# JoshuaLim007/Software-Raytracer

Hardware: AMD Instinct MI355X
Metric: path-samples/sec at 1920x1080x8-bounce; achieved HBM GB/s vs peak (higher is better)
Workload: dtype f32; 1 GPU; BASELINE config 2: Scene1.json 1920x1080, 32 spp, 8 bounces, FOV 55, camera at origin; workload_key=Scene1 1920x1080 rows0-1080 spp32 b8, partition=single frame

## Files before the change

### software-raytracer_amd/csrc/srt_capi.hip

```cpp
#include <hip/hip_runtime.h>
#include <math.h>
#include <stdarg.h>
#include <stddef.h>
#include <stdio.h>
#include <stdlib.h>
#include <string.h>

#include <algorithm>
#include <exception>
#include <new>
#include <vector>

#include "srt_kernel.hip.h"
#include "srt_gbuffer.hip.h"
#include "srt_denoise.hip.h"
#include "srt_temporal.hip.h"
#include "srt_upsample.hip.h"
#include "srt_antialias.hip.h"
#include "srt_variance.hip.h"
#include "srt_moments.hip.h"
#include "srt_refit.hip.h"
#include "srt_rays.hip.h"
#include "srt_outputs_host.h"
#include "srt_rays_host.h"
// ... 1111 lines not shown
template <int MIN_WAVES, bool MESH>
static void launch_pathtrace(bool tally, bool in_lds, bool multi, bool defer, dim3 grid, size_t lds_bytes, hipStream_t stream, const srt::KernelParams& K) {
    using srt::pathtrace_kernel;
    void (*const kernel)(srt::KernelParams) =
        tally && defer    ? pathtrace_kernel<MIN_WAVES, MESH, true, false, true, false, true>
        : tally && multi  ? pathtrace_kernel<MIN_WAVES, MESH, true, true, false, false, true>
        : tally           ? pathtrace_kernel<MIN_WAVES, MESH, true, false, false, false, true>
        : in_lds && defer ? pathtrace_kernel<MIN_WAVES, MESH, true, false, true>
        : in_lds && multi ? pathtrace_kernel<MIN_WAVES, MESH, true, true, false>
        : in_lds          ? pathtrace_kernel<MIN_WAVES, MESH, true, false, false>
        : defer           ? pathtrace_kernel<MIN_WAVES, MESH, false, false, true>
        : multi           ? pathtrace_kernel<MIN_WAVES, MESH, false, true, false>
                          : pathtrace_kernel<MIN_WAVES, MESH, false, false, false>;
    hipLaunchKernelGGL(kernel, grid, dim3(srt::WG_THREADS), lds_bytes, stream, K);
}

static void launch_pathtrace_rows(bool tally, bool six, dim3 grid, size_t lds_bytes, hipStream_t stream, const srt::KernelParams& K) {
    using srt::pathtrace_kernel;
    void (*const kernel)(srt::KernelParams) =
        tally ? pathtrace_kernel<5, false, true, false, false, false, true, true>
        : six ? pathtrace_kernel<6, false, true, false, false, false, false, true>
              : pathtrace_kernel<5, false, true, false, false, false, false, true>;
    hipLaunchKernelGGL(kernel, grid, dim3(srt::WG_THREADS), lds_bytes, stream, K);
}

static int launch_render(srt_context* ctx, const srt_render_params* p, srt::KernelParams& K, const KernelSetup& ks, const RenderLaunch& L) {
    const bool in_lds = ctx->scene_in_lds[ks.img];
    const bool want_work = (p->flags & SRT_RENDER_COUNT_WORK) != 0;
    const bool rule_applies = (p->sample_count >= 64 || K.n_tris > 0) && p->sample_count >= 32 && K.steps <= 1;
    const bool tally = ((L.record && rule_applies) || want_work) && in_lds;
    ctx->count_work = want_work;
    ctx->count_work_valid = want_work && tally;
    if (tally && want_work) {
        SRT_HIP(ctx, hipMemsetAsync(ctx->d_work, 0, srt::TALLY_ALL * sizeof(unsigned long long), ctx->stream));
        K.work_counter = ctx->d_work;
    }
    const bool timing = !(p->flags & SRT_RENDER_NO_TIMING);
    if (timing) SRT_HIP(ctx, hipEventRecord(ctx->ev_begin, ctx->stream));
    const bool multi = L.shape.tile_h < srt::TILE_H || (K.steps > 1 && !(K.flags & SRT_RENDER_PREVIEW)) || L.bgrid;
    if (K.n_tris > 0)
        launch_pathtrace<4, true>(tally, in_lds, multi, L.defer, L.grid, ks.lds_bytes, ctx->stream, K);
#ifdef SRT_DEV
    else if (ks.use == 1 && in_lds && !multi && !L.defer && !tally)
        hipLaunchKernelGGL((srt::pathtrace_kernel<4, false>), L.grid, dim3(srt::WG_THREADS), ks.lds_bytes, ctx->stream, K);
    else if (ks.use == 3 && in_lds && !multi && !L.defer && !tally)
        hipLaunchKernelGGL((srt::pathtrace_kernel<3, false>), L.grid, dim3(srt::WG_THREADS), ks.lds_bytes, ctx->stream, K);
#endif
    else if (L.rows) {
        const size_t rows_lds = ks.lds_bytes - (size_t)(srt::WG_SCRATCH_BYTES - srt::WG_SCRATCH_BYTES_ROWS);
        bool six = srt::rows_six_waves(rows_lds);
#ifdef SRT_DEV
        if (ks.use == 5) six = false;
#endif
        launch_pathtrace_rows(tally, six, L.grid, rows_lds, ctx->stream, K);
    }
    else
        launch_pathtrace<5, false>(tally, in_lds, multi, L.defer, L.grid, ks.lds_bytes, ctx->stream, K);
    if (L.defer) {
        SRT_HIP(ctx, hipGetLastError());
        hipLaunchKernelGGL(srt::fold_kernel, dim3((unsigned)L.shape.wg8), dim3(256), 0, ctx->stream, K, (int)L.shape.wg_x);
    }
    SRT_HIP(ctx, hipGetLastError());
    if (timing) SRT_HIP(ctx, hipEventRecord(ctx->ev_end, ctx->stream));
    ctx->pending_timed = timing;
    if (L.record) {
        const size_t nwg = (size_t)L.grid.x * L.grid.y;
        SRT_HIP(ctx, hipMemcpyAsync(ctx->h_wg_cost, ctx->d_wg_cost, REC_WORDS * nwg * 4, hipMemcpyDeviceToHost, ctx->stream));
        SRT_HIP(ctx, hipEventRecord(ctx->ev_cost, ctx->stream));
        ctx->recording = true;
        ctx->rec_gx = L.grid.x, ctx->rec_gy = L.grid.y;
        ctx->rec_has_work = tally;
        ctx->rec_step_w = probe_step_weight(K, ProbeWeights());
        ctx->order_stale = false;
    }
    return SRT_OK;
}

static void note_pending(srt_context* ctx, const srt_render_params* p, const srt::KernelParams& K, const RenderLaunch& L) {
    ctx->launched = true;
    ctx->stats_pending = true;
    ctx->pending_samples = (uint64_t)ctx->width * (uint64_t)K.rows * p->sample_count;
    ctx->pending_chunks = (uint32_t)L.shape.chunks;
    ctx->pending_tile_rows = (uint32_t)L.shape.tile_h;
    ctx->pending_chunk_samples = L.defer ? (uint32_t)L.shape.chunk : 0u;
    ctx->pending_shape_source = L.shape.source;
    ctx->work_layout[0] = K.nu, ctx->work_layout[1] = K.nc, ctx->work_layout[2] = K.K, ctx->work_layout[3] = K.nb;
}

extern "C" {

int srt_render(srt_context* ctx, const srt_render_params* p) {
    if (const int rc = check_render_params(ctx, p)) return rc;
    SRT_HIP(ctx, hipSetDevice(ctx->device));
    srt::KernelParams K;
    const KernelSetup ks = fill_kernel_params(ctx, p, K);
    ctx->count_rays = (p->flags & SRT_RENDER_COUNT_RAYS) != 0;
    if (ctx->count_rays) SRT_HIP(ctx, hipMemsetAsync(ctx->d_rays, 0, sizeof(unsigned long long), ctx->stream));
    RenderLaunch L;
    if (const int rc = enter_band(ctx, K)) return rc;
    if (const int rc = plan_launch(ctx, p, K, ks, L)) return rc;
    if (const int rc = plan_cost_order(ctx, p, K, ks, L)) return rc;
    if (const int rc = launch_render(ctx, p, K, ks, L)) return rc;
    note_pending(ctx, p, K, L);
    return SRT_OK;
}

#ifdef SRT_DEV
// ... 1182 lines not shown
```

### software-raytracer_amd/csrc/srt_kernel.hip.h

```cpp
#pragma once

#include <hip/hip_runtime.h>
#include <stdint.h>

#include <type_traits>

#include "srt_defs.h"
#include "srt_launch_shape.h"

namespace srt {

struct KernelParams {
    float cam_pos[3];
    float right_rd[3];
    float up_ld[3];
    float fwd_clip[3];
    int32_t width, height;
    int32_t y0, rows;
    uint32_t first_sample, sample_count;
    int32_t max_bounces;
    uint32_t seed, flags;
    int32_t steps, stripe_width, selected;
    int32_t bgrid_w, bgrid_h;
    int32_t nu4, nc, K, nsT, nb;
    int32_t nu;
    int32_t off_bounds, off_box, off_mat;
    int32_t scene_vec4;
    const float4* scene;
    const float4* bvh_nodes;
    const float4* bvh_tris;
    const int32_t* bvh_gidpos;
    int32_t n_tris;
    float mesh_center[3];
    float mesh_half[3];
    float mesh_r1;
    float mesh_bs_radius;
    int32_t mesh_defer;
    int32_t mesh_wait;
    int32_t tile_h;
    int32_t chunk;
    int32_t chunk_full;
    float4* sample_rows;
    unsigned long long* tile_masks;
    uint32_t* tile_chain;
    int32_t chunk_layers;
    const uint32_t* wg_order;
    uint32_t* wg_cost;
    uint32_t wg_blocks;
    unsigned long long* work_counter;
    float4* accumulator;
    uint32_t* framebuffer;
    unsigned long long* ray_counter;
#ifdef SRT_DEV
    int32_t chain_mode;
    uint32_t chain_arg;
#endif
};

#ifdef SRT_DEV
enum : int32_t {
    DEV_CHAIN_NATURAL = 0,
    DEV_CHAIN_OFF = 1,
    DEV_CHAIN_CUT = 2,
    DEV_CHAIN_TILES = 3,
};
__host__ __device__ inline uint32_t dev_chain_cut(int32_t mode, uint32_t arg, uint32_t layers, uint32_t tile) {
    if (mode == DEV_CHAIN_CUT) return arg < layers ? arg : layers;
    if (mode == DEV_CHAIN_TILES) return srt_mix32(srt_mix32(arg ^ 0x9E3779B9u) + tile) % (layers + 1u);
    if (mode == DEV_CHAIN_OFF) return 0u;
    return layers;
}
#endif

constexpr uint32_t KF_BLOCK_GRID = 0x10u;
constexpr uint32_t KF_BOXES_FINITE = 0x20u;
constexpr uint32_t SRT_MESH_ORDER_W = 6u;
constexpr int TILE_W = 8, TILE_H = 8;
constexpr int WG_TILES_X = 2, WG_TILES_Y = 2;
constexpr int WG_THREADS = 64 * WG_TILES_X * WG_TILES_Y;
constexpr int WG_W = TILE_W * WG_TILES_X, WG_H = TILE_H * WG_TILES_Y;
struct TilePixel {
    int lx, ly, x, y;
};
__device__ __forceinline__ TilePixel tile_pixel() {
    const int lane = threadIdx.x & 63, wave = threadIdx.x >> 6;
    TilePixel t;
    t.lx = (wave % WG_TILES_X) * TILE_W + (lane & 7), t.ly = (wave / WG_TILES_X) * TILE_H + (lane >> 3);
    t.x = (int)blockIdx.x * WG_W + t.lx, t.y = (int)blockIdx.y * WG_H + t.ly;
    return t;
}
constexpr int WORK_MAX = 512;
constexpr int RING_DEPTH = 2;
constexpr int WAVE_RING_BYTES = 64 * RING_DEPTH * 16;
constexpr int WAVE_SCRATCH_BYTES = 64 * 8 + WORK_MAX * 2 + 64 * 12 * 4 + WAVE_RING_BYTES;
constexpr int WG_SCRATCH_BYTES = WAVE_SCRATCH_BYTES * WG_TILES_X * WG_TILES_Y;
constexpr int ROWS_IN_FLIGHT = 8;
constexpr int WG_SCRATCH_BYTES_ROWS = (WAVE_SCRATCH_BYTES - WAVE_RING_BYTES) * WG_TILES_X * WG_TILES_Y;
constexpr int MESH_Q = 512;
constexpr float MESH_T_MIN_CULL = 0.0099f;
#ifdef SRT_STATS
__device__ unsigned long long g_stats[8];
#define SRT_STAT(i, v) do { if (__builtin_amdgcn_mbcnt_hi(~0u, __builtin_amdgcn_mbcnt_lo(~0u, 0u)) == 0) atomicAdd(&g_stats[i], (unsigned long long)(v)); } while (0)
#else
#define SRT_STAT(i, v) do { } while (0)
#endif
// ... 835 lines not shown

__device__ __forceinline__ void accumulate_sample(const KernelParams& P, float4& acc, RGB c, float a, uint32_t sidx) {
    const uint32_t frame = P.first_sample + sidx;
    if (sidx == 0 && (P.flags & 1u) != 0) {
        acc = make_float4(c.r, c.g, c.b, a);
    } else {
        float weight = frame <= 16777216u ? div_window(1.0f, (float)(int)frame) : (float)(1.0 / (double)(int)frame);
        float om = 1 - weight;
        acc.x = clamp0(acc.x * om) + c.r * weight;
        acc.y = clamp0(acc.y * om) + c.g * weight;
        acc.z = clamp0(acc.z * om) + c.b * weight;
        acc.w = clamp0(acc.w * om) + a * weight;
    }
}
__device__ __forceinline__ uint32_t tone_map(const float4 acc) {
    float r = acc.x / (1.0f + acc.x);
    float g = acc.y / (1.0f + acc.y);
    float b = acc.z / (1.0f + acc.z);
    float a = acc.w / (0.0f + acc.w);
    return pack_channel(a) << 24 | pack_channel(r) << 16 | pack_channel(g) << 8 | pack_channel(b);
}
__device__ __forceinline__ void store_framebuffer(uint32_t* framebuffer, int x, int y, int W, int H, const float4 r) {
    if (framebuffer) framebuffer[(size_t)(H - 1 - y) * W + x] = tone_map(r);
}
__device__ __forceinline__ void store_result(float4* dst, size_t p, uint32_t* framebuffer, int x, int y, int W, int H, const float4 r) {
    dst[p] = r;
    store_framebuffer(framebuffer, x, y, W, H, r);
}
__device__ __forceinline__ void store_pixel(const KernelParams& P, uint32_t pix, const float4 acc) {
    P.accumulator[pix] = acc;
    const uint32_t px = tone_map(acc);
    const uint32_t py = pix / (uint32_t)P.width, pxx = pix - py * (uint32_t)P.width;
    P.framebuffer[(size_t)(P.height - 1 - (int)py) * P.width + pxx] = px;
}

template <bool SCENE_LDS, bool ROWS = false>
__device__ __forceinline__ Lds make_lds(const KernelParams& P, float4* lds, int waves, int wave) {
    constexpr int stride = WAVE_SCRATCH_BYTES - (ROWS ? WAVE_RING_BYTES : 0);
    char* wg = reinterpret_cast<char*>(lds + (SCENE_LDS ? P.scene_vec4 : 0));
    char* scratch = wg + wave * stride;
    const float4* image;
    if constexpr (SCENE_LDS)
        image = lds;
    else
        image = P.scene;
    return Lds{image, image + CONST_ROWS, P.nu4, P.nu, P.nc, P.K, P.nsT, P.nb, P.off_bounds, P.off_box, P.off_mat,
               reinterpret_cast<unsigned long long*>(scratch), reinterpret_cast<unsigned short*>(scratch + 64 * 8),
               reinterpret_cast<float*>(scratch + 64 * 8 + WORK_MAX * 2),
               reinterpret_cast<float4*>(scratch + 64 * 8 + WORK_MAX * 2 + 64 * 12 * 4),
               reinterpret_cast<unsigned*>(wg + waves * stride + wave * MESH_WAVE_BYTES)};
}

template <int MIN_WAVES, bool MESH, bool SCENE_LDS = true, bool MULTI = false, bool DEFER = false, bool PROBE = false, bool TALLY_ = false, bool ROWS = false>
__global__ void __launch_bounds__(WG_THREADS, MIN_WAVES) pathtrace_kernel(const KernelParams P) {
    static_assert(!PROBE || (!MULTI && !DEFER), "the probe runs the full-tile pool");
    static_assert(!ROWS || (!MULTI && !DEFER && !PROBE), "rows of the sample buffer: one chunk, full tiles, a real launch");
    constexpr bool TALLY = TALLY_ || PROBE;
    extern __shared__ float4 lds_scene[];
    Tally<TALLY> tally{};
#if defined(SRT_STATS) && SRT_STATS == 3
    Prof prof;
    prof.last = (long long)__builtin_readcyclecounter();
    for (int i = 0; i < 8; ++i) prof.acc[i] = 0;
#endif
    if constexpr (SCENE_LDS) {
        constexpr int STAGE = 8;
        const int n = P.scene_vec4;
        float4 row[STAGE];
#pragma unroll
        for (int k = 0; k < STAGE; ++k) {
            const int i = (int)threadIdx.x + k * WG_THREADS;
            row[k] = i < n ? P.scene[i] : make_float4(0, 0, 0, 0);
        }
#pragma unroll
        for (int k = 0; k < STAGE; ++k) {
            const int i = (int)threadIdx.x + k * WG_THREADS;
            if (i < n) lds_scene[i] = row[k];
        }
        for (int i = (int)threadIdx.x + STAGE * WG_THREADS; i < n; i += WG_THREADS) lds_scene[i] = P.scene[i];
        __syncthreads();
    }
    const Lds S = make_lds<SCENE_LDS, ROWS>(P, lds_scene, WG_TILES_X * WG_TILES_Y, threadIdx.x >> 6);
    if (PROBE && (threadIdx.x >> 6) != 0) return;

    const int lane = threadIdx.x & 63, wave = threadIdx.x >> 6;
    const int tile_h = P.tile_h;
#if defined(SRT_STATS) && SRT_STATS == 6
    const long long t_start = (long long)__builtin_readcyclecounter();
    const unsigned long long r_start = __builtin_amdgcn_s_memrealtime();
    const unsigned hw_start = __builtin_amdgcn_s_getreg(0xF804), xcc_start = __builtin_amdgcn_s_getreg(0xF814);
#elif defined(SRT_STATS) && SRT_STATS == 5
    const long long t_start = (long long)__builtin_readcyclecounter();
#else
    const long long t_start = !PROBE && P.wg_cost ? (long long)__builtin_amdgcn_s_memrealtime() : 0;
#endif
    uint32_t block_id = blockIdx.y * gridDim.x + blockIdx.x;
    if (P.wg_order) block_id = P.wg_order[block_id];
    const int bx = (int)(block_id % gridDim.x), by = (int)(block_id / gridDim.x);
    const int tx = bx * WG_W + (lane & (TILE_W - 1)) * WG_TILES_X + (wave % WG_TILES_X);
    const int ty = by * (tile_h * WG_TILES_Y) + (lane / TILE_W) * WG_TILES_Y + (wave / WG_TILES_X);
    const int W = P.width, H = P.height;
    const bool bgrid = MULTI && (P.flags & KF_BLOCK_GRID) != 0;
    bool in_range_;
    int x_, y_, ax, ay;
    if (bgrid) {
        const int sw = P.stripe_width > 0 ? P.stripe_width : W;
        const int per_stripe = (sw + P.steps - 1) / P.steps;
        const int stripe = tx / per_stripe;
        ax = stripe * sw + (tx - stripe * per_stripe) * P.steps;
        ay = (P.y0 / P.steps + ty) * P.steps;
        in_range_ = tx < P.bgrid_w && ty < P.bgrid_h && ax < W && ay < P.y0 + P.rows && (lane / TILE_W) < tile_h;
        if (!in_range_) ax = 0, ay = (P.y0 / P.steps) * P.steps;
        x_ = ax, y_ = ay;
    } else {
        in_range_ = tx < W && ty < P.rows && (lane / TILE_W) < tile_h;
        x_ = in_range_ ? tx : 0, y_ = in_range_ ? (P.y0 + ty) : P.y0;
        ax = x_, ay = y_;
        if (P.steps > 1) {
            const int s0 = P.stripe_width > 0 ? (x_ / P.stripe_width) * P.stripe_width : 0;
            ax = s0 + ((x_ - s0) / P.steps) * P.steps;
            ay = (y_ / P.steps) * P.steps;
        }
    }
    const bool in_range = in_range_;
    const int x = x_, y = y_;
    const uint32_t pixel = (uint32_t)(x + y * W);
    const uint32_t rng_pixel = (uint32_t)(ax + ay * W);
    auto write_blocks = [&](bool have, int bx0, int by0, float4 val, bool keep) {
        const unsigned long long m = __builtin_amdgcn_ballot_w64(have);
        if (m == 0ull) return;
        const int n = __builtin_popcountll(m);
        const int rank = (int)__builtin_amdgcn_mbcnt_hi((unsigned)(m >> 32), __builtin_amdgcn_mbcnt_lo((unsigned)m, 0u));
        float4* sv = S.ring;
        unsigned* sa = reinterpret_cast<unsigned*>(S.work);
        __builtin_amdgcn_wave_barrier();
        if (have) {
            sv[rank] = val;
            sa[rank] = (unsigned)bx0, sa[64 + rank] = (unsigned)by0;
            sa[128 + rank] = keep ? 0u : tone_map(val);
        }
        __builtin_amdgcn_wave_barrier();
        const int steps = P.steps, per = steps * steps;
        const int L = per < 64 ? per : 64, G = 64 / L;
        const int g = lane / L, ql = lane - g * L;
        for (int b0 = 0; b0 < n; b0 += G) {
            const int b = b0 + g;
            const bool on = g < G && b < n;
            const int bi = on ? b : 0;
            const int x0 = (int)sa[bi], y0b = (int)sa[64 + bi];
            const float4 v = sv[bi];
            const uint32_t px = sa[128 + bi];
// ... 5 lines not shown
            x_end = x_end < W ? x_end : W;
            int y_hi = y0b + steps;
            y_hi = y_hi < P.y0 + P.rows ? y_hi : P.y0 + P.rows;
            for (int q = ql; q < per; q += 64) {
                const int j = q / steps, i = q - j * steps;
                const int xx = x0 + i, yy = y0b + j;
                if (on && xx < x_end && yy >= P.y0 && yy < y_hi) {
                    const uint32_t pp = (uint32_t)(xx + yy * W);
                    if (keep) {
                        float4 a = P.accumulator[pp];
                        accumulate_sample(P, a, RGB{v.x, v.y, v.z}, tag_alpha(__float_as_uint(v.w)), 0);
                        P.accumulator[pp] = a;
                        P.framebuffer[(size_t)(H - 1 - yy) * W + xx] = tone_map(a);
                    } else {
                        P.accumulator[pp] = v;
                        P.framebuffer[(size_t)(H - 1 - yy) * W + xx] = px;
                    }
                }
            }
        }
        __builtin_amdgcn_wave_barrier();
    };
    int lead_lane = lane;
    if constexpr (MULTI) {
        if (P.steps > 1 && !(P.flags & 4u) && !bgrid) {
            const uint32_t key = in_range ? rng_pixel : 0xFFFFFFFFu - (uint32_t)lane;
            unsigned long long same = 0ull;
            for (int i = 0; i < 64; ++i)
                if ((uint32_t)__builtin_amdgcn_readlane((int)key, i) == key) same |= 1ull << i;
            lead_lane = __builtin_ctzll(same);
        }
    }
    const bool is_leader = lead_lane == lane;

    float nX = ((float)ax / (float)W) * 2 - 1;
    float nY = ((float)ay / (float)H) * 2 - 1;
    V3 u = v3(P.right_rd[0] * nX, P.right_rd[1] * nX, P.right_rd[2] * nX);
    V3 vv = v3(P.up_ld[0] * nY, P.up_ld[1] * nY, P.up_ld[2] * nY);
    const V3 dir0 = normalized(v3((u.x + vv.x) + P.fwd_clip[0], (u.y + vv.y) + P.fwd_clip[1], (u.z + vv.z) + P.fwd_clip[2]));
    const V3 cam = v3(P.cam_pos[0], P.cam_pos[1], P.cam_pos[2]);

    bool parked = false;
    const Hit h0 = closest_hit<MESH, TALLY, SCENE_LDS>(S, P, cam, dir0, true, 1, parked, tally SRT_PROF_ARG);

    const bool reset = (P.flags & 1u) != 0;
    uint32_t s_base = 0u, count = P.sample_count;
    if constexpr (DEFER) {
        const uint32_t z = blockIdx.z, zf = (uint32_t)P.chunk_full, S = (uint32_t)P.chunk, half = S >> 1;
        s_base = SRT_CHUNK_FIRST(z, S, zf, half);
        const uint32_t want = z < zf ? S : half;
        count = P.sample_count - s_base < want ? P.sample_count - s_base : want;
    }
    const int B = P.max_bounces;
    unsigned rays = 0;

    auto accumulate = [&](float4& acc, RGB c, float a, uint32_t sidx) { accumulate_sample(P, acc, c, a, sidx); };
    auto write_pixel = [&](uint32_t pix, const float4 acc) { store_pixel(P, pix, acc); };

    const bool preview = (P.flags & 4u) != 0;
    const bool pix_traced = in_range && h0.prim >= 0 && B > 0 && !preview;
    const bool traced = pix_traced && is_leader;
    float4 untraced_val = make_float4(0, 0, 0, 0);
    tally.add(TALLY_UNTRACED_WAVES, __builtin_amdgcn_ballot_w64(in_range && !pix_traced) != 0ull ? 1u : 0u);
    tally.add(TALLY_WAVES, 1u);
    if (!PROBE && in_range && !pix_traced && (!DEFER || blockIdx.z == 0)) {
        RGB c;
        float ca = 0.0f;
        if (h0.prim < 0) {
            c = environment(S, dir0);
            ca = environment_alpha(dir0);
        } else if (preview) {
            float4 m0 = S.mat(h0.prim, 0), m1 = S.mat(h0.prim, 1);
            float k2 = 2 * dot3(dir0, h0.n);
            const V3 rd = v3(dir0.x - h0.n.x * k2, dir0.y - h0.n.y * k2, dir0.z - h0.n.z * k2);
            RGB refl = environment(S, rd);
            const float k = m0.y, sm = m0.x;
            float fresnal = 0;
            if (S.order(h0.prim) == P.selected) {
                fresnal = 1 - dot3(v3(h0.n.x * -1, h0.n.y * -1, h0.n.z * -1), dir0);
                fresnal = tmax(fresnal, 0.0f);
                if (fresnal < 0.0f) {
                    fresnal = 0;
                } else if (fresnal >= 0.5f) {
                    fresnal = 1;
                } else {
                    fresnal = (fresnal - 0.0f) / (0.5f - 0.0f);
                    fresnal = fresnal * fresnal * (3 - 2 * fresnal);
                }
            }
            RGB base{clamp0(m0.z), clamp0(m0.w), clamp0(m1.x)}, emis{clamp0(m1.y), clamp0(m1.z), clamp0(m1.w)};
            const float omk = 1 - k;
            RGB a{clamp0(clamp0(clamp0(base.r * omk) + clamp0(clamp0(refl.r * k) * sm)) + emis.r),
                  clamp0(clamp0(clamp0(base.g * omk) + clamp0(clamp0(refl.g * k) * sm)) + emis.g),
                  clamp0(clamp0(clamp0(base.b * omk) + clamp0(clamp0(refl.b * k) * sm)) + emis.b)};
            c = color_lerp(a, RGB{3.0f, 3.0f, 0.0f}, fresnal);
            const float aa = clamp0(clamp0(clamp0(0.0f * omk) + clamp0(clamp0(environment_alpha(rd) * k) * sm)) + 0.0f);
            ca = clamp0(aa * (1 - fresnal) + 0.0f * fresnal);
        } else {
            float4 m1 = S.mat(h0.prim, 1);
            c = RGB{clamp0(m1.y), clamp0(m1.z), clamp0(m1.w)};
        }
        if (bgrid) {
            untraced_val = make_float4(c.r, c.g, c.b, __uint_as_float(alpha_tag(ca)));
            if (reset) {
                untraced_val = make_float4(0, 0, 0, 0);
                for (uint32_t i = 0; i < P.sample_count; ++i) accumulate(untraced_val, c, ca, i);
            }
        } else {
            float4 acc = reset ? make_float4(0, 0, 0, 0) : P.accumulator[pixel];
            for (uint32_t i = 0; i < P.sample_count; ++i) accumulate(acc, c, ca, i);
            write_pixel(pixel, acc);
        }
        if (is_leader) rays += P.sample_count;
    }
    if constexpr (MULTI) {
        if (bgrid) write_blocks(in_range && !pix_traced, ax, ay, untraced_val, !reset);
    }

    const unsigned long long hitmask = __builtin_amdgcn_ballot_w64(traced);
    const size_t tile_id = (size_t)block_id * (WG_TILES_X * WG_TILES_Y) + wave;
    if (DEFER && blockIdx.z == 0 && lane == 0) P.tile_masks[tile_id] = hitmask;
    const int n_hit = __builtin_popcountll(hitmask);
    if (n_hit > 0) {
        float* rec = S.pix;
        if (traced) {
            const int slot = (int)__builtin_amdgcn_mbcnt_hi((unsigned)(hitmask >> 32), __builtin_amdgcn_mbcnt_lo((unsigned)hitmask, 0u));
            float* r = rec + slot * 12;
            r[0] = dir0.x, r[1] = dir0.y, r[2] = dir0.z;
            r[3] = h0.n.x, r[4] = h0.n.y, r[5] = h0.n.z;
            r[6] = h0.p.x, r[7] = h0.p.y, r[8] = h0.p.z;
            r[9] = __int_as_float(h0.prim);
            r[10] = __uint_as_float(srt_mix32(srt_mix32(P.seed ^ 0xA511E9B3U) + rng_pixel));
            r[11] = __uint_as_float(pixel);
        }
        constexpr int ring_depth = RING_DEPTH;
        const int depth = (64 * ring_depth) / n_hit;
        const bool depth_pow2 = (depth & (depth - 1)) == 0;
        auto ring_row = [&](uint32_t s) { return depth_pow2 ? (s & (uint32_t)(depth - 1)) : (s % (uint32_t)depth); };
        float4* ring = S.ring;
        if constexpr (!ROWS)
            for (int i = lane; i < 64 * ring_depth; i += 64) ring[i] = make_float4(0, 0, 0, __uint_as_float(0xFFFFFFFFu));
        __builtin_amdgcn_wave_barrier();

        const bool owner = lane < n_hit;
        uint32_t own_pixel = 0, own_done = owner ? 0u : count;
        float4 acc = make_float4(0, 0, 0, 0);
        const bool blocks = MULTI && P.steps > 1 && !(P.flags & 4u) && !bgrid;
        const bool bgrid_keep = bgrid && !reset;
        const bool fold_px = blocks && pix_traced;
        const int fslot = __builtin_popcountll(hitmask & ((1ull << lead_lane) - 1ull));
        uint32_t fdone = fold_px ? 0u : count;
        if (blocks) {
            if (fold_px && !reset) acc = P.accumulator[pixel];
        } else if (!ROWS && owner) {
            own_pixel = __float_as_uint(rec[lane * 12 + 11]);
            if (!DEFER && !reset && !bgrid) acc = P.accumulator[own_pixel];
        }
        bool chained = false;
        if constexpr (DEFER) {
            if (P.tile_chain) {
                const uint32_t at = blockIdx.z == 0 ? 0u : (uint32_t)__builtin_amdgcn_readfirstlane((int)coherent_load(P.tile_chain + tile_id));
                chained = at == blockIdx.z;
#ifdef SRT_DEV
                chained = chained && blockIdx.z < dev_chain_cut(P.chain_mode, P.chain_arg, gridDim.z, (uint32_t)tile_id);
#endif
                if (chained && owner && (blockIdx.z > 0 || !reset)) acc = coherent_load(P.accumulator + own_pixel);
            }
        }

        bool busy = false;
        uint32_t task = 0;
        RGB L{0, 0, 0}, T{0, 0, 0};
        V3 sray = v3(0, 0, 1), hn = v3(0, 0, 0), hp = v3(0, 0, 0);
        int hprim = 0, bounce = 0;
        float spec = 0.0f;
        uint32_t rng = 0;

        uint32_t own_next = own_done;
        int rot = 0;
        unsigned handed = 0;
        const int fold_pace = (63 + n_hit) / n_hit;
        int park_steps = 0;

        while (true) {
            SRT_TICK(7);
            if constexpr (ROWS) {
                if (__builtin_amdgcn_ballot_w64(busy || own_next < count) == 0ull) break;
            } else {
            const bool drain = __builtin_amdgcn_ballot_w64(busy) == 0ull || __builtin_amdgcn_ballot_w64(own_next < count) == 0ull;
            const int fold_its = drain || fold_pace > depth ? depth : fold_pace;
            for (int it = 0; it < fold_its; ++it) {
                bool ready = false;
                float4 e = make_float4(0, 0, 0, 0);
                if (own_done < count) {
                    e = ring[ring_row(own_done) * n_hit + lane];
                    ready = (__float_as_uint(e.w) & ~TAG_ALPHA_NAN) == own_done;
                }
                if constexpr (MULTI) {
                    if (blocks) {
                        bool ready_px = false;
                        float4 f = make_float4(0, 0, 0, 0);
                        if (fdone < count) {
                            f = ring[ring_row(fdone) * n_hit + fslot];
                            ready_px = (__float_as_uint(f.w) & ~TAG_ALPHA_NAN) == fdone;
                        }
                        if (__builtin_amdgcn_ballot_w64(ready | ready_px) == 0ull) break;
                        if (ready_px) {
                            accumulate(acc, RGB{f.x, f.y, f.z}, tag_alpha(__float_as_uint(f.w)), fdone);
                            ++fdone;
                        }
                        if (ready) ++own_done;
                        continue;
                    }
                }
                const unsigned long long readym = __builtin_amdgcn_ballot_w64(ready);
                if (readym == 0ull) break;
#if defined(SRT_STATS) && SRT_STATS == 4
                {
                    const int st_ready = __builtin_popcountll(readym);
                    SRT_STAT(4, 1);
                    SRT_STAT(5, st_ready);
                }
#endif
                if (it == 0 && !drain && __builtin_popcountll(readym) * 5 < n_hit &&
                    __builtin_amdgcn_ballot_w64(own_next < count && own_next >= own_done + (uint32_t)depth) == 0ull)
                    break;
                if (ready) {
                    if (DEFER && chained)
                        accumulate(acc, RGB{e.x, e.y, e.z}, tag_alpha(__float_as_uint(e.w)), s_base + own_done);
                    else if constexpr (DEFER)
                        P.sample_rows[(tile_id * P.sample_count + s_base + own_done) * 64 + lane] = e;
                    else if (MULTI && bgrid_keep)
                        acc = e;
                    else
                        accumulate(acc, RGB{e.x, e.y, e.z}, tag_alpha(__float_as_uint(e.w)), own_done);
                    ++own_done;
                }
            }
            if (__builtin_amdgcn_ballot_w64(own_done < count) == 0ull) break;
            }
// ... 88 lines not shown
            tally.add(TALLY_STEPS, 1u);
            V3 o = v3(0, 0, 0);
            const float ofs = .00001f;
            if (MESH && busy && parked) {
                o = v3(hp.x + hn.x * ofs, hp.y + hn.y * ofs, hp.z + hn.z * ofs);
            } else if (busy) {
                if (bounce != 0) {
                    T = RGB{T.r * 0.8f, T.g * 0.8f, T.b * 0.8f};
                }
                float k2 = 2 * dot3(sray, hn);
                V3 refl = v3(sray.x - hn.x * k2, sray.y - hn.y * k2, sray.z - hn.z * k2);
                uint32_t r0 = srt_mix32(rng) >> 17;
                uint32_t r1 = srt_mix32(rng + 0x9E3779B9U) >> 17;
                uint32_t r2 = srt_mix32(rng + 2u * 0x9E3779B9U) >> 17;
                rng += 3u * 0x9E3779B9U;
                V3 sr = v3((rand_unit(r0) - 0.5f) * 2, (rand_unit(r1) - 0.5f) * 2,
                           (rand_unit(r2) - 0.5f) * 2);
                sr = normalized_in_window(sr);
                if (dot3(sr, hn) < 0) sr = v3(sr.x * -1, sr.y * -1, sr.z * -1);
                float tt = S.mat(hprim, 0).x * spec;
                V3 l = v3(sr.x * (1 - tt) + refl.x * tt, sr.y * (1 - tt) + refl.y * tt, sr.z * (1 - tt) + refl.z * tt);
                sray = normalized(l);
                o = v3(hp.x + hn.x * ofs, hp.y + hn.y * ofs, hp.z + hn.z * ofs);
            }
            const Hit h = closest_hit<MESH, TALLY, SCENE_LDS>(S, P, o, sray, busy, MESH && park_steps >= P.mesh_wait ? 1 : P.mesh_defer, parked, tally SRT_PROF_ARG);
            if constexpr (MESH) park_steps = __builtin_amdgcn_ballot_w64(busy && parked) != 0ull ? park_steps + 1 : 0;
            if (busy && !(MESH && parked)) {
                ++rays;
                bool end_path;
                uint32_t atag = 0u;
                if (h.prim < 0) {
                    RGB e = environment(S, sray);
                    L = RGB{L.r + e.r * T.r, L.g + e.g * T.g, L.b + e.b * T.b};
                    atag = alpha_tag(environment_alpha(sray));
                    end_path = true;
                } else {
                    float4 m0 = S.mat(h.prim, 0), m1 = S.mat(h.prim, 1), m2 = S.mat(h.prim, 2);
                    uint32_t r = srt_mix32(rng) >> 17;
                    rng += 0x9E3779B9U;
                    spec = (m0.y >= rand_unit(r)) ? 1.0f : 0.0f;
                    RGB Em{m1.y, m1.z, m1.w};
                    L = RGB{L.r + Em.r * T.r, L.g + Em.g * T.g, L.b + Em.b * T.b};
                    RGB Bc{m0.z, m0.w, m1.x}, Sc{m2.x, m2.y, m2.z};
                    const float ns = 1 - spec;
                    RGB f{Bc.r * ns + Sc.r * spec, Bc.g * ns + Sc.g * spec, Bc.b * ns + Sc.b * spec};
                    T = RGB{T.r * f.r, T.g * f.g, T.b * f.b};
                    hn = h.n;
                    hp = h.p;
                    hprim = h.prim;
                    ++bounce;
                    end_path = bounce >= B;
                }
                if (end_path) {
                    const uint32_t sidx = task >> 6;
                    const float4 e = make_float4(L.r, L.g, L.b, __uint_as_float(sidx | atag));
                    if constexpr (ROWS)
                        P.sample_rows[tile_id * count * 64 + task] = e;
                    else
                        ring[ring_row(sidx) * n_hit + (int)(task & 63u)] = e;
                    busy = false;
                }
            }
            __builtin_amdgcn_wave_barrier();
        }
        if constexpr (ROWS) {
            SRT_TICK(7);
            __builtin_amdgcn_fence(__ATOMIC_RELEASE, "workgroup");
            __builtin_amdgcn_fence(__ATOMIC_ACQUIRE, "workgroup");
            if (owner) {
                own_pixel = __float_as_uint(rec[lane * 12 + 11]);
                if (!reset) acc = P.accumulator[own_pixel];
                const float4* row = P.sample_rows + tile_id * count * 64 + lane;
                uint32_t s = 0;
                for (; s + ROWS_IN_FLIGHT <= count; s += ROWS_IN_FLIGHT) {
                    float4 c[ROWS_IN_FLIGHT];
#pragma unroll
                    for (int k = 0; k < ROWS_IN_FLIGHT; ++k) c[k] = row[(size_t)(s + k) * 64];
#pragma unroll
                    for (int k = 0; k < ROWS_IN_FLIGHT; ++k) accumulate(acc, RGB{c[k].x, c[k].y, c[k].z}, tag_alpha(__float_as_uint(c[k].w)), s + k);
                }
                for (; s < count; ++s) {
                    const float4 c = row[(size_t)s * 64];
                    accumulate(acc, RGB{c.x, c.y, c.z}, tag_alpha(__float_as_uint(c.w)), s);
                }
                write_pixel(own_pixel, acc);
            }
            SRT_TICK(0);
        } else if (blocks) {
            if (fold_px) write_pixel(pixel, acc);
        } else if (MULTI && bgrid) {
            const int oy = (int)(own_pixel / (uint32_t)W), ox = (int)(own_pixel - (uint32_t)oy * (uint32_t)W);
            write_blocks(owner, ox, oy, acc, bgrid_keep);
        } else if (!DEFER && !PROBE && owner) {
            write_pixel(own_pixel, acc);
        }
        if constexpr (DEFER) {
            if (chained) {
                if (owner) {
                    if (blockIdx.z + 1 == gridDim.z) write_pixel(own_pixel, acc);
                    else coherent_store(P.accumulator + own_pixel, acc);
                }
                asm volatile("s_waitcnt vmcnt(0)" ::: "memory");
                if (lane == 0) coherent_store(P.tile_chain + tile_id, (uint32_t)blockIdx.z + 1u);
            }
        }
    }

#if defined(SRT_STATS) && SRT_STATS == 3
    SRT_TICK(7);
    for (int i = 0; i < 8; ++i) SRT_STAT(i, prof.acc[i] > 0 ? prof.acc[i] : 0);
#endif
#if defined(SRT_STATS) && SRT_STATS == 5
    SRT_STAT(7, (long long)__builtin_readcyclecounter() - t_start);
#endif
#if defined(SRT_STATS) && SRT_STATS == 6
    {
        const long long t_end = (long long)__builtin_readcyclecounter();
        const unsigned long long r_end = __builtin_amdgcn_s_memrealtime();
        const unsigned hw_end = __builtin_amdgcn_s_getreg(0xF804), xcc_end = __builtin_amdgcn_s_getreg(0xF814);
        const size_t w = ((size_t)(blockIdx.z * gridDim.y + blockIdx.y) * gridDim.x + blockIdx.x) * (WG_TILES_X * WG_TILES_Y) + wave;
        if (lane == 0 && w < (size_t)WAVE_LOG_MAX) {
            unsigned long long* e = g_wave_log + 6 * w;
            e[0] = (unsigned long long)t_start, e[1] = (unsigned long long)t_end, e[2] = r_start, e[3] = r_end;
            e[4] = (unsigned long long)hw_start | ((unsigned long long)xcc_start << 32), e[5] = (unsigned long long)hw_end | ((unsigned long long)xcc_end << 32);
        }
    }
#endif
    if constexpr (PROBE) {
        if (lane < TALLY_N && tally.v) atomicAdd(&P.wg_cost[(size_t)block_id * TALLY_N + lane], tally.v);
        return;
    }
    if constexpr (TALLY) {
        if (P.work_counter && lane < TALLY_ALL && tally.v) atomicAdd(&P.work_counter[lane], (unsigned long long)tally.v);
    }
    if ((P.flags & 2u) || P.wg_cost) {
        unsigned long long tot = rays;
        for (int off = 32; off > 0; off >>= 1) tot += __shfl_down(tot, off);
        if (lane == 0 && tot) {
            if (P.flags & 2u) atomicAdd(P.ray_counter, tot);
            if (P.wg_cost) {
                const long long dt = (long long)__builtin_amdgcn_s_memrealtime() - t_start;
                atomicAdd(&P.wg_cost[block_id], (dt > 0 && dt < (1ll << 28)) ? (uint32_t)dt : (uint32_t)(tot < (1ull << 24) ? tot * 16ull : (1ull << 28)));
            }
        }
        if constexpr (TALLY) if (P.wg_cost && lane < TALLY_N && tally.v) {
            uint32_t* rec = P.wg_cost + P.wg_blocks + ((size_t)block_id * (WG_TILES_X * WG_TILES_Y) + wave) * TALLY_N;
            atomicAdd(&rec[lane], tally.v);
        }
    }
}


__global__ void __launch_bounds__(256) fold_kernel(const KernelParams P, int tiles_x_wg) {
    const int lane = threadIdx.x & 63, wave = threadIdx.x >> 6;
    const size_t wg = blockIdx.x;
    const size_t tile_id = wg * (WG_TILES_X * WG_TILES_Y) + wave;
    const unsigned long long mask = P.tile_masks[tile_id];
    const int n_hit = __builtin_popcountll(mask);
    if (lane >= n_hit) return;
    unsigned long long m = mask;
    for (int i = 0; i < lane; ++i) m &= m - 1ull;
    const int bit = __builtin_ctzll(m);
    const int bx = (int)(wg % (size_t)tiles_x_wg), by = (int)(wg / (size_t)tiles_x_wg);
    const int x = bx * WG_W + (bit & (TILE_W - 1)) * WG_TILES_X + (wave % WG_TILES_X);
    const int y = P.y0 + by * WG_H + (bit / TILE_W) * WG_TILES_Y + (wave / WG_TILES_X);
    const uint32_t pixel = (uint32_t)(x + y * P.width);
    uint32_t first = 0u;
    if (P.tile_chain) {
        const uint32_t at = P.tile_chain[tile_id];
        if (at >= (uint32_t)P.chunk_layers) return;
        first = chunk_first(at, (uint32_t)P.chunk, (uint32_t)P.chunk_full);
    }
    float4 acc = ((P.flags & 1u) && first == 0u) ? make_float4(0, 0, 0, 0) : P.accumulator[pixel];
    const float4* row = P.sample_rows + tile_id * P.sample_count * 64 + lane;
    const uint32_t n = P.sample_count;
    uint32_t s = first;
    for (; s + 8 <= n; s += 8) {
        float4 c[8];
#pragma unroll
        for (int k = 0; k < 8; ++k) c[k] = row[(size_t)(s + k) * 64];
#pragma unroll
        for (int k = 0; k < 8; ++k) accumulate_sample(P, acc, RGB{c[k].x, c[k].y, c[k].z}, tag_alpha(__float_as_uint(c[k].w)), s + k);
    }
    for (; s < n; ++s) {
        const float4 c = row[(size_t)s * 64];
        accumulate_sample(P, acc, RGB{c.x, c.y, c.z}, tag_alpha(__float_as_uint(c.w)), s);
    }
    store_pixel(P, pixel, acc);
}

__global__ void __launch_bounds__(256) selftest_normalize_kernel(uint32_t seed, unsigned long long first, unsigned long long n, unsigned long long* mismatches) {
    const unsigned long long i = (unsigned long long)blockIdx.x * 256ull + threadIdx.x;
    const unsigned wave_kind = (unsigned)((i >> 6) & 3ull);
    uint32_t h = srt_mix32(seed ^ (uint32_t)i) + (uint32_t)(i >> 32) * 0x9E3779B9U;
    auto next = [&]() { h = srt_mix32(h + 0x9E3779B9U); return h; };
    auto any_float = [&](unsigned kind) {
        const uint32_t r = next();
        switch (kind) {
            case 0: return __uint_as_float((r & 0x807FFFFFu) | ((100u + (next() % 56u)) << 23));
            case 1: return __uint_as_float(r);
            case 2: return __uint_as_float((r & 0x807FFFFFu) | ((next() % 255u) << 23));
// ... 218 lines not shown
```

### software-raytracer_amd/csrc/srt_launch_shape.h

```cpp
#pragma once

#include <math.h>
#include <stddef.h>
#include <stdint.h>

#include <algorithm>
#include <vector>

namespace srt {

constexpr int SHAPE_TILE_H = 8, SHAPE_WG_W = 16, SHAPE_WG_H = 16, SHAPE_WG_TILES_Y = 2, SHAPE_WAVES_PER_WG = 4;
constexpr int SHAPE_TALLY_N = 8;

struct BlockWork {
    float sum, longest;
};

struct RecordWeights {
    double group, node_test, mesh_phase, wave;
};
constexpr RecordWeights k_record_weights_analytic{110.0, 0.0, 0.0, 2500.0};
constexpr RecordWeights k_record_weights_mesh{127.0, 34.0, 33.0, 6900.0};

struct WorkRecord {
// ... 119 lines not shown

#define SRT_CHUNK_FIRST(z, chunk, chunk_full, half) ((z) < (chunk_full) ? (z) * (chunk) : (chunk_full) * (chunk) + ((z) - (chunk_full)) * (half))
#ifdef __HIPCC__
#define SRT_SHAPE_HD __host__ __device__
#else
#define SRT_SHAPE_HD
#endif
SRT_SHAPE_HD inline uint32_t chunk_first(uint32_t z, uint32_t chunk, uint32_t chunk_full) {
    return SRT_CHUNK_FIRST(z, chunk, chunk_full, chunk >> 1);
}
SRT_SHAPE_HD inline uint32_t chunk_count(uint32_t z, uint32_t chunk, uint32_t chunk_full, uint32_t sample_count) {
    const uint32_t first = chunk_first(z, chunk, chunk_full), want = z < chunk_full ? chunk : chunk >> 1;
    return sample_count - first < want ? sample_count - first : want;
}
#undef SRT_SHAPE_HD

inline void shape_without_sample_buffer(LaunchShape& s) {
    s.chunk = 0, s.chunks = 1, s.chunk_full = 1;
}

inline void finish_launch_shape(LaunchShape& s, uint32_t sample_count, const ShapeOverrides& ov = ShapeOverrides()) {
    if (s.chunks < 2) return;
    s.tile_h = SHAPE_TILE_H;
    s.chunk_full = s.chunks;
    const int taper = s.chunks >= 4 ? 2 : 1;
    if (s.chunk >= 24 && !ov.no_taper) {
        const int half = s.chunk >> 1, full = s.chunks - taper;
        const long long rest = (long long)sample_count - (long long)full * s.chunk;
        s.chunk_full = full;
        s.chunks = full + (int)((rest + half - 1) / half);
    }
}

constexpr uint32_t ROWS_MIN_SAMPLES = 2;
constexpr unsigned long long ROWS_MAX_BYTES = 4ull << 30;
inline bool fold_from_rows(const LaunchShape& s, const ShapeRequest& q, bool preview, bool scene_in_lds) {
    if (s.chunks >= 2 || s.tile_h != SHAPE_TILE_H || q.block_grid || q.steps > 1 || preview) return false;
    if (q.mesh || !scene_in_lds) return false;
    if (q.sample_count < ROWS_MIN_SAMPLES || s.wg8 < 1) return false;
    return (unsigned long long)s.wg8 <= ROWS_MAX_BYTES / 1024ull / q.sample_count / SHAPE_WAVES_PER_WG;
}
inline unsigned long long rows_bytes(const LaunchShape& s, uint32_t sample_count) {
    return (unsigned long long)s.wg8 * SHAPE_WAVES_PER_WG * sample_count * 1024ull;
}

constexpr size_t SHAPE_ROWS_WG_SCRATCH_BYTES = 18432;
constexpr size_t LDS_BYTES_PER_CU = 160 * 1024, LDS_GRANULE_BYTES = 1280;
inline bool rows_six_waves(size_t lds_bytes) {
    if (lds_bytes > LDS_BYTES_PER_CU) return false;
    const size_t held = (lds_bytes + LDS_GRANULE_BYTES - 1) / LDS_GRANULE_BYTES * LDS_GRANULE_BYTES;
    return 6 * held <= LDS_BYTES_PER_CU;
}

}
```

Measured before the change: 36.65 billion path-samples/s.

## Chain row-buffer tiles in persistent workgroups, carrying in-flight paths across tiles

In the rows path-trace mode each workgroup now processes a chain of up to two tiles, and the grid shrinks to match. Paths still in flight when a tile's own samples run out are not drained to completion. Their state goes to LDS and the next tile's sample rows, and they finish while the next tile's work runs, so the drain tail at the end of each tile is hidden. This also saves a scene-to-LDS staging per chained tile. In exchange the code grows more complex, the kernel uses more registers, fold and accounting are deferred across links, and the kernel params are read through the kernarg pointer.

Result: slower. 33.85 billion path-samples/s (-7.7%).

```diff
diff --git a/software-raytracer_amd/csrc/srt_capi.hip b/software-raytracer_amd/csrc/srt_capi.hip
--- a/software-raytracer_amd/csrc/srt_capi.hip
+++ b/software-raytracer_amd/csrc/srt_capi.hip
@@ -1187,7 +1187,14 @@
 #ifdef SRT_DEV
         if (ks.use == 5) six = false;
 #endif
-        launch_pathtrace_rows(tally, six, L.grid, rows_lds, ctx->stream, K);
+        const long long blocks = (long long)L.grid.x * L.grid.y;
+        int chain = srt::rows_chain(blocks, (long long)ctx->cu_count * (six ? 6 : 5));
+#ifdef SRT_DEV
+        if (ks.use > 20 && ks.use <= 28) chain = ks.use - 20;
+#endif
+        K.chain_len = chain, K.blocks_x = (int32_t)L.grid.x, K.chain_blocks = (uint32_t)blocks;
+        const dim3 grid = chain > 1 ? dim3((unsigned)((blocks + chain - 1) / chain)) : L.grid;
+        launch_pathtrace_rows(tally, six, grid, rows_lds, ctx->stream, K);
     }
     else
         launch_pathtrace<5, false>(tally, in_lds, multi, L.defer, L.grid, ks.lds_bytes, ctx->stream, K);
diff --git a/software-raytracer_amd/csrc/srt_kernel.hip.h b/software-raytracer_amd/csrc/srt_kernel.hip.h
--- a/software-raytracer_amd/csrc/srt_kernel.hip.h
+++ b/software-raytracer_amd/csrc/srt_kernel.hip.h
@@ -51,6 +51,9 @@
     float4* accumulator;
     uint32_t* framebuffer;
     unsigned long long* ray_counter;
+    int32_t chain_len;
+    int32_t blocks_x;
+    uint32_t chain_blocks;
 #ifdef SRT_DEV
     int32_t chain_mode;
     uint32_t chain_arg;
@@ -992,7 +995,8 @@
 }
 
 template <int MIN_WAVES, bool MESH, bool SCENE_LDS = true, bool MULTI = false, bool DEFER = false, bool PROBE = false, bool TALLY_ = false, bool ROWS = false>
-__global__ void __launch_bounds__(WG_THREADS, MIN_WAVES) pathtrace_kernel(const KernelParams P) {
+__global__ void __launch_bounds__(WG_THREADS, MIN_WAVES) pathtrace_kernel(const KernelParams P_arg) {
+    const KernelParams& P = P_arg;
     static_assert(!PROBE || (!MULTI && !DEFER), "the probe runs the full-tile pool");
     static_assert(!ROWS || (!MULTI && !DEFER && !PROBE), "rows of the sample buffer: one chunk, full tiles, a real launch");
     constexpr bool TALLY = TALLY_ || PROBE;
@@ -1023,7 +1027,7 @@
     const Lds S = make_lds<SCENE_LDS, ROWS>(P, lds_scene, WG_TILES_X * WG_TILES_Y, threadIdx.x >> 6);
     if (PROBE && (threadIdx.x >> 6) != 0) return;
 
-    const int lane = threadIdx.x & 63, wave = threadIdx.x >> 6;
+    const int lane_id = threadIdx.x & 63, wave = ROWS ? __builtin_amdgcn_readfirstlane((int)(threadIdx.x >> 6)) : (int)(threadIdx.x >> 6);
     const int tile_h = P.tile_h;
 #if defined(SRT_STATS) && SRT_STATS == 6
     const long long t_start = (long long)__builtin_readcyclecounter();
@@ -1034,9 +1038,39 @@
 #else
     const long long t_start = !PROBE && P.wg_cost ? (long long)__builtin_amdgcn_s_memrealtime() : 0;
 #endif
-    uint32_t block_id = blockIdx.y * gridDim.x + blockIdx.x;
-    if (P.wg_order) block_id = P.wg_order[block_id];
-    const int bx = (int)(block_id % gridDim.x), by = (int)(block_id / gridDim.x);
+    static_assert(ROWS_MIN_SAMPLES >= 2, "a carried path's registers wait in the first two rows of the next tile");
+    constexpr uint32_t TASK_PREV = 0x80000000u, TASK_BUSY = 0x40000000u;
+    const uint32_t wg_pos = blockIdx.y * gridDim.x + blockIdx.x, wg_count = gridDim.x * gridDim.y;
+    const int links = ROWS && P.chain_len > 1 ? P.chain_len : 1;
+    [[maybe_unused]] long long t_link = t_start;
+    [[maybe_unused]] unsigned rays_told = 0;
+    [[maybe_unused]] uint32_t prev_block = 0;
+    [[maybe_unused]] unsigned long long prev_mask = 0ull;
+    [[maybe_unused]] uint32_t next_block = ROWS && P.wg_order ? P.wg_order[wg_pos] : wg_pos;
+    unsigned rays = 0;
+    bool busy = false;
+    uint32_t task = 0;
+    RGB L{0, 0, 0}, T{0, 0, 0};
+    V3 sray = v3(0, 0, 1), hn = v3(0, 0, 0), hp = v3(0, 0, 0);
+    int hprim = 0, bounce = 0;
+    float spec = 0.0f;
+    uint32_t rng = 0;
+    for (int link = 0;; ++link) {
+    const KernelParams* P_link = &P_arg;
+    int lane_ = lane_id;
+    if constexpr (ROWS) {
+        auto kp = __builtin_amdgcn_kernarg_segment_ptr();
+        asm volatile("" : "+s"(kp));
+        P_link = (const KernelParams*)kp;
+        asm volatile("" : "+v"(lane_));
+    }
+    const KernelParams& P = *P_link;
+    const int lane = lane_;
+    uint32_t block_id = ROWS ? next_block : blockIdx.y * gridDim.x + blockIdx.x;
+    const bool last_link = !ROWS || link + 1 >= links || wg_pos + (uint32_t)(link + 1) * wg_count >= P.chain_blocks;
+    if (!ROWS && P.wg_order) block_id = P.wg_order[block_id];
+    const uint32_t blocks_x = ROWS ? (uint32_t)P.blocks_x : gridDim.x;
+    const int bx = (int)(block_id % blocks_x), by = (int)(block_id / blocks_x);
     const int tx = bx * WG_W + (lane & (TILE_W - 1)) * WG_TILES_X + (wave % WG_TILES_X);
     const int ty = by * (tile_h * WG_TILES_Y) + (lane / TILE_W) * WG_TILES_Y + (wave / WG_TILES_X);
     const int W = P.width, H = P.height;
@@ -1148,7 +1182,6 @@
         count = P.sample_count - s_base < want ? P.sample_count - s_base : want;
     }
     const int B = P.max_bounces;
-    unsigned rays = 0;
 
     auto accumulate = [&](float4& acc, RGB c, float a, uint32_t sidx) { accumulate_sample(P, acc, c, a, sidx); };
     auto write_pixel = [&](uint32_t pix, const float4 acc) { store_pixel(P, pix, acc); };
@@ -1215,9 +1248,25 @@
 
     const unsigned long long hitmask = __builtin_amdgcn_ballot_w64(traced);
     const size_t tile_id = (size_t)block_id * (WG_TILES_X * WG_TILES_Y) + wave;
+    [[maybe_unused]] const size_t prev_tile = (size_t)prev_block * (WG_TILES_X * WG_TILES_Y) + wave;
+    if constexpr (ROWS) {
+        const float* st = S.pix + lane * 12;
+        asm volatile("" : "+v"(st));
+        L = RGB{st[0], st[1], st[2]}, T = RGB{st[3], st[4], st[5]};
+        hn = v3(st[6], st[7], st[8]), hp = v3(st[9], st[10], st[11]);
+        const float4* gs = P.sample_rows + tile_id * count * 64 + lane;
+        asm volatile("" : "+v"(gs));
+        const float4 g0 = gs[0], g1 = gs[64];
+        sray = v3(g0.x, g0.y, g0.z), spec = g0.w;
+        hprim = __float_as_int(g1.x), bounce = __float_as_int(g1.y), rng = __float_as_uint(g1.z), task = __float_as_uint(g1.w);
+        busy = link > 0 && (task & TASK_BUSY) != 0u;
+        task &= ~TASK_BUSY;
+        __builtin_amdgcn_wave_barrier();
+    }
     if (DEFER && blockIdx.z == 0 && lane == 0) P.tile_masks[tile_id] = hitmask;
     const int n_hit = __builtin_popcountll(hitmask);
-    if (n_hit > 0) {
+    if (n_hit > 0 || (ROWS && __builtin_amdgcn_ballot_w64(busy) != 0ull)) {
+        const int n_div = ROWS && n_hit == 0 ? 1 : n_hit;
         float* rec = S.pix;
         if (traced) {
             const int slot = (int)__builtin_amdgcn_mbcnt_hi((unsigned)(hitmask >> 32), __builtin_amdgcn_mbcnt_lo((unsigned)hitmask, 0u));
@@ -1230,7 +1279,7 @@
             r[11] = __uint_as_float(pixel);
         }
         constexpr int ring_depth = RING_DEPTH;
-        const int depth = (64 * ring_depth) / n_hit;
+        const int depth = (64 * ring_depth) / n_div;
         const bool depth_pow2 = (depth & (depth - 1)) == 0;
         auto ring_row = [&](uint32_t s) { return depth_pow2 ? (s & (uint32_t)(depth - 1)) : (s % (uint32_t)depth); };
         float4* ring = S.ring;
@@ -1264,24 +1313,16 @@
             }
         }
 
-        bool busy = false;
-        uint32_t task = 0;
-        RGB L{0, 0, 0}, T{0, 0, 0};
-        V3 sray = v3(0, 0, 1), hn = v3(0, 0, 0), hp = v3(0, 0, 0);
-        int hprim = 0, bounce = 0;
-        float spec = 0.0f;
-        uint32_t rng = 0;
-
         uint32_t own_next = own_done;
         int rot = 0;
         unsigned handed = 0;
-        const int fold_pace = (63 + n_hit) / n_hit;
+        const int fold_pace = (63 + n_div) / n_div;
         int park_steps = 0;
 
         while (true) {
             SRT_TICK(7);
             if constexpr (ROWS) {
-                if (__builtin_amdgcn_ballot_w64(busy || own_next < count) == 0ull) break;
+                if (__builtin_amdgcn_ballot_w64((busy && (last_link || (task & TASK_PREV) != 0u)) || own_next < count) == 0ull) break;
             } else {
             const bool drain = __builtin_amdgcn_ballot_w64(busy) == 0ull || __builtin_amdgcn_ballot_w64(own_next < count) == 0ull;
             const int fold_its = drain || fold_pace > depth ? depth : fold_pace;
@@ -1476,10 +1517,11 @@
                     end_path = bounce >= B;
                 }
                 if (end_path) {
-                    const uint32_t sidx = task >> 6;
+                    const uint32_t own_task = ROWS ? task & ~TASK_PREV : task;
+                    const uint32_t sidx = own_task >> 6;
                     const float4 e = make_float4(L.r, L.g, L.b, __uint_as_float(sidx | atag));
                     if constexpr (ROWS)
-                        P.sample_rows[tile_id * count * 64 + task] = e;
+                        P.sample_rows[((task & TASK_PREV) != 0u ? prev_tile : tile_id) * count * 64 + own_task] = e;
                     else
                         ring[ring_row(sidx) * n_hit + (int)(task & 63u)] = e;
                     busy = false;
@@ -1488,13 +1530,53 @@
             __builtin_amdgcn_wave_barrier();
         }
         if constexpr (ROWS) {
-            SRT_TICK(7);
-            __builtin_amdgcn_fence(__ATOMIC_RELEASE, "workgroup");
-            __builtin_amdgcn_fence(__ATOMIC_ACQUIRE, "workgroup");
-            if (owner) {
-                own_pixel = __float_as_uint(rec[lane * 12 + 11]);
-                if (!reset) acc = P.accumulator[own_pixel];
-                const float4* row = P.sample_rows + tile_id * count * 64 + lane;
+        } else if (blocks) {
+            if (fold_px) write_pixel(pixel, acc);
+        } else if (MULTI && bgrid) {
+            const int oy = (int)(own_pixel / (uint32_t)W), ox = (int)(own_pixel - (uint32_t)oy * (uint32_t)W);
+            write_blocks(owner, ox, oy, acc, bgrid_keep);
+        } else if (!DEFER && !PROBE && owner) {
+            write_pixel(own_pixel, acc);
+        }
+        if constexpr (DEFER) {
+            if (chained) {
+                if (owner) {
+                    if (blockIdx.z + 1 == gridDim.z) write_pixel(own_pixel, acc);
+                    else coherent_store(P.accumulator + own_pixel, acc);
+                }
+                asm volatile("s_waitcnt vmcnt(0)" ::: "memory");
+                if (lane == 0) coherent_store(P.tile_chain + tile_id, (uint32_t)blockIdx.z + 1u);
+            }
+        }
+    }
+    if constexpr (ROWS) {
+        if (!last_link) {
+            const uint32_t pos = wg_pos + (uint32_t)(link + 1) * wg_count;
+            next_block = P.wg_order ? P.wg_order[pos] : pos;
+            if (busy) task |= TASK_PREV | TASK_BUSY;
+            float* st = S.pix + lane * 12;
+            st[0] = L.r, st[1] = L.g, st[2] = L.b, st[3] = T.r, st[4] = T.g, st[5] = T.b;
+            st[6] = hn.x, st[7] = hn.y, st[8] = hn.z, st[9] = hp.x, st[10] = hp.y, st[11] = hp.z;
+            float4* gs = P.sample_rows + ((size_t)next_block * (WG_TILES_X * WG_TILES_Y) + wave) * count * 64 + lane;
+            gs[0] = make_float4(sray.x, sray.y, sray.z, spec);
+            gs[64] = make_float4(__int_as_float(hprim), __int_as_float(bounce), __uint_as_float(rng), __uint_as_float(task));
+            busy = false;
+        }
+        SRT_TICK(7);
+        __builtin_amdgcn_fence(__ATOMIC_RELEASE, "workgroup");
+        __builtin_amdgcn_fence(__ATOMIC_ACQUIRE, "workgroup");
+        for (int f = prev_mask != 0ull ? 0 : 1; f < (last_link ? 2 : 1); ++f) {
+            const uint32_t f_block = f == 0 ? prev_block : block_id;
+            const unsigned long long f_mask = f == 0 ? prev_mask : hitmask;
+            if ((f_mask >> lane) & 1ull) {
+                const int slot = (int)__builtin_amdgcn_mbcnt_hi((unsigned)(f_mask >> 32), __builtin_amdgcn_mbcnt_lo((unsigned)f_mask, 0u));
+                const int f_bx = (int)(f_block % blocks_x), f_by = (int)(f_block / blocks_x);
+                const int f_x = f_bx * WG_W + (lane & (TILE_W - 1)) * WG_TILES_X + (wave % WG_TILES_X);
+                const int f_y = P.y0 + f_by * (tile_h * WG_TILES_Y) + (lane / TILE_W) * WG_TILES_Y + (wave / WG_TILES_X);
+                const uint32_t f_pixel = (uint32_t)(f_x + f_y * W);
+                float4 acc = make_float4(0, 0, 0, 0);
+                if (!reset) acc = P.accumulator[f_pixel];
+                const float4* row = P.sample_rows + ((size_t)f_block * (WG_TILES_X * WG_TILES_Y) + wave) * count * 64 + slot;
                 uint32_t s = 0;
                 for (; s + ROWS_IN_FLIGHT <= count; s += ROWS_IN_FLIGHT) {
                     float4 c[ROWS_IN_FLIGHT];
@@ -1507,27 +1589,11 @@
                     const float4 c = row[(size_t)s * 64];
                     accumulate(acc, RGB{c.x, c.y, c.z}, tag_alpha(__float_as_uint(c.w)), s);
                 }
-                write_pixel(own_pixel, acc);
-            }
-            SRT_TICK(0);
-        } else if (blocks) {
-            if (fold_px) write_pixel(pixel, acc);
-        } else if (MULTI && bgrid) {
-            const int oy = (int)(own_pixel / (uint32_t)W), ox = (int)(own_pixel - (uint32_t)oy * (uint32_t)W);
-            write_blocks(owner, ox, oy, acc, bgrid_keep);
-        } else if (!DEFER && !PROBE && owner) {
-            write_pixel(own_pixel, acc);
-        }
-        if constexpr (DEFER) {
-            if (chained) {
-                if (owner) {
-                    if (blockIdx.z + 1 == gridDim.z) write_pixel(own_pixel, acc);
-                    else coherent_store(P.accumulator + own_pixel, acc);
-                }
-                asm volatile("s_waitcnt vmcnt(0)" ::: "memory");
-                if (lane == 0) coherent_store(P.tile_chain + tile_id, (uint32_t)blockIdx.z + 1u);
-            }
-        }
+                write_pixel(f_pixel, acc);
+            }
+        }
+        prev_block = block_id, prev_mask = hitmask;
+        SRT_TICK(0);
     }
 
 #if defined(SRT_STATS) && SRT_STATS == 3
@@ -1554,6 +1620,26 @@
         if (lane < TALLY_N && tally.v) atomicAdd(&P.wg_cost[(size_t)block_id * TALLY_N + lane], tally.v);
         return;
     }
+    if constexpr (ROWS) {
+        if constexpr (TALLY) {
+            if (P.work_counter && lane < TALLY_ALL && tally.v) atomicAdd(&P.work_counter[lane], (unsigned long long)tally.v);
+            if (P.wg_cost && lane < TALLY_N && tally.v) atomicAdd(&(P.wg_cost + P.wg_blocks + tile_id * TALLY_N)[lane], tally.v);
+            tally.v = 0u;
+        }
+        if (P.wg_cost || ((P.flags & 2u) && last_link)) {
+            unsigned long long tot = rays;
+            for (int off = 32; off > 0; off >>= 1) tot += __shfl_down(tot, off);
+            if (P.wg_cost) {
+                const long long now = (long long)__builtin_amdgcn_s_memrealtime(), dt = now - t_link;
+                const unsigned told = (unsigned)__builtin_amdgcn_readfirstlane((int)(unsigned)tot), here = told - rays_told;
+                if (lane == 0 && here) atomicAdd(&P.wg_cost[block_id], (dt > 0 && dt < (1ll << 28)) ? (uint32_t)dt : (here < (1u << 24) ? here * 16u : (1u << 28)));
+                t_link = now, rays_told = told;
+            }
+            if ((P.flags & 2u) && last_link && lane == 0 && tot) atomicAdd(P.ray_counter, tot);
+        }
+        if (last_link) break;
+        continue;
+    }
     if constexpr (TALLY) {
         if (P.work_counter && lane < TALLY_ALL && tally.v) atomicAdd(&P.work_counter[lane], (unsigned long long)tally.v);
     }
@@ -1571,6 +1657,8 @@
             uint32_t* rec = P.wg_cost + P.wg_blocks + ((size_t)block_id * (WG_TILES_X * WG_TILES_Y) + wave) * TALLY_N;
             atomicAdd(&rec[lane], tally.v);
         }
+    }
+    break;
     }
 }
 
diff --git a/software-raytracer_amd/csrc/srt_launch_shape.h b/software-raytracer_amd/csrc/srt_launch_shape.h
--- a/software-raytracer_amd/csrc/srt_launch_shape.h
+++ b/software-raytracer_amd/csrc/srt_launch_shape.h
@@ -195,4 +195,13 @@
     return 6 * held <= LDS_BYTES_PER_CU;
 }
 
-}
+constexpr int ROWS_CHAIN_MAX = 2;
+constexpr long long ROWS_CHAIN_ROUNDS = 2;
+inline int rows_chain(long long blocks, long long resident) {
+    if (blocks < 1 || resident < 1) return 1;
+    for (int k = ROWS_CHAIN_MAX; k > 1; --k)
+        if ((blocks + k - 1) / k >= ROWS_CHAIN_ROUNDS * resident) return k;
+    return 1;
+}
+
+}
```
